# liuzuxin/OSRL

Measured on AMD Instinct MI355X. Metric: grad-steps/sec, higher is better.
Workload: dtype f32

## Files before the change

### osrl_amd/csrc/dwt.h

```cpp
#pragma once
#include "mlp_common.h"

namespace {

template <int T>
struct DwFragT {
  f32x4 a[T], b[T];
};

template <int T>
__device__ __forceinline__ void dwt_load(DwFragT<T>& f, const float* __restrict__ pz, const float* __restrict__ pa,
                                         size_t ldz, size_t lda_g, const unsigned (&oa)[T], const unsigned (&ia)[T],
                                         int nob, int nib) {
#pragma unroll
  for (int t = 0; t < 4; ++t) {
#pragma unroll
    for (int ob = 0; ob < T; ++ob) f.a[ob][t] = pz[t * ldz + oa[ob]];
#pragma unroll
    for (int ib = 0; ib < T; ++ib) f.b[ib][t] = pa[t * lda_g + ia[ib]];
  }
}
template <int T>
__device__ __forceinline__ void dwt_load_tail(DwFragT<T>& f, const float* __restrict__ dz, const float* __restrict__ av,
                                              size_t ldz, size_t lda_g, const unsigned (&oa)[T], const unsigned (&ia)[T],
                                              int nob, int nib, int r0, int r_end, int kq) {
#pragma unroll
  for (int t = 0; t < 4; ++t) {
    const int r = r0 + 4 * kq + t;
    const bool rok = r < r_end;
    const size_t rc = (size_t)(rok ? r : r_end - 1);
#pragma unroll
    for (int ob = 0; ob < T; ++ob) {
      const float v = dz[rc * ldz + oa[ob]];
      f.a[ob][t] = rok ? v : 0.f;
    }
#pragma unroll
    for (int ib = 0; ib < T; ++ib) f.b[ib][t] = av[rc * lda_g + ia[ib]];
  }
}

template <int T, int SHAPE>
__device__ __forceinline__ void dwt_mma(f32x4 (&acc)[T][T], float (&dbacc)[T], const DwFragT<T>& f, int nob, int nib,
                                        bool want_db) {
  constexpr bool FULL = SHAPE == 1;
#pragma unroll
  for (int t = 0; t < 4; ++t) {
#pragma unroll
    for (int ob = 0; ob < (SHAPE == 2 ? 1 : T); ++ob) {
      if (SHAPE != 0 || ob < nob) {
#pragma unroll
        for (int ib = 0; ib < T; ++ib)
          if (SHAPE != 0 || ib < nib) acc[ob][ib] = __builtin_amdgcn_mfma_f32_16x16x4f32(f.a[ob][t], f.b[ib][t], acc[ob][ib], 0, 0, 0);
      }
    }
  }
  (void)FULL;
  if (want_db) {
#pragma unroll
    for (int ob = 0; ob < T; ++ob) dbacc[ob] += (f.a[ob][0] + f.a[ob][1]) + (f.a[ob][2] + f.a[ob][3]);
  }
}

template <int T>
constexpr size_t dwt_lds() { return sizeof(float) * (4 * (16 * T) * (16 * T + 1) + 4 * 16 * T); }

template <int T, bool WARM = false, bool DEEP = false, class EPI>
__device__ __forceinline__ void dwt_tile(const osrl_dw_entry_t* __restrict__ entries, const int32_t* __restrict__ items,
                                         const int item, const int rows, float* __restrict__ red, EPI epi) {
  constexpr int TW = 16 * T, LD = TW + 1;
  const int tid = threadIdx.x, lane = tid & 63;
  const int wave = __builtin_amdgcn_readfirstlane(tid >> 6);
  const int ei = items[item * 4 + 0], ot = items[item * 4 + 1], it = items[item * 4 + 2], sp = items[item * 4 + 3];
  const int s = sp & 0xffff, nsp = sp >> 16;
  const OSRL_CAS osrl_dw_entry_t& E = ((const OSRL_CAS osrl_dw_entry_t*)entries)[ei];
  const int out = E.out, in = E.in;
  const size_t ldz = E.ldz > 0 ? (size_t)E.ldz : (size_t)out, lda_g = E.lda > 0 ? (size_t)E.lda : (size_t)in;
  const int o0 = ot * TW, i0 = it * TW;
  int rps = (rows + nsp - 1) / nsp;
  rps = (rps + 63) & ~63;
  const int rpw = rps >> 2;
  const int r_begin = s * rps + wave * rpw;
  int r_end = r_begin + rpw;
  r_end = r_end > rows ? rows : r_end;
  const int m = lane & 15, kq = lane >> 4;
  int nob = (out - o0 + 15) >> 4;
  nob = nob > T ? T : nob;
  int nib = (in - i0 + 15) >> 4;
  nib = nib > T ? T : nib;
  const bool want_db = it == 0;

  if (wave < 4) {
  f32x4 acc[T][T];
  zero_acc<T, T>(acc);
  float dbacc[T];
#pragma unroll
  for (int ob = 0; ob < T; ++ob) dbacc[ob] = 0.f;
  const float* __restrict__ dz = E.dz;
  const float* __restrict__ av = E.a;
  unsigned oa[T], ia[T];
#pragma unroll
  for (int b = 0; b < T; ++b) {
    const int o = o0 + b * 16 + m, i = i0 + b * 16 + m;
    oa[b] = (unsigned)(o < out ? o : 0);
    ia[b] = (unsigned)(i < in ? i : 0);
  }
  if (r_begin < r_end) {
    const int n_full = (r_end - r_begin) >> 4;
    const float* __restrict__ pz = dz + (size_t)(r_begin + 4 * kq) * ldz;
    const float* __restrict__ pa = av + (size_t)(r_begin + 4 * kq) * lda_g;
    float wt[WARM ? 4 * ((TW + 31) / 32) : 1];
    if constexpr (WARM) {
      constexpr int NL = (TW + 31) / 32;
#pragma unroll
      for (int pass = 0; pass < 2; ++pass) {
        int r = r_begin + pass * 64 + lane;
        r = r < r_end ? r : r_end - 1;
#pragma unroll
        for (int j = 0; j < NL; ++j) {
          const int oc = o0 + 32 * j < out ? o0 + 32 * j : out - 1, ic = i0 + 32 * j < in ? i0 + 32 * j : in - 1;
          wt[(pass * 2 + 0) * NL + j] = dz[(size_t)r * ldz + oc];
          wt[(pass * 2 + 1) * NL + j] = av[(size_t)r * lda_g + ic];
        }
      }
    }
    DwFragT<T> f0, f1;
    auto run = [&](auto full_c) {
      constexpr int FULL = decltype(full_c)::value;
      if constexpr (DEEP) {
        if (n_full == 4 && r_begin + 64 == r_end) {
          DwFragT<T> f2, f3;
          dwt_load<T>(f0, pz, pa, ldz, lda_g, oa, ia, nob, nib);
          dwt_load<T>(f1, pz + (size_t)16 * ldz, pa + (size_t)16 * lda_g, ldz, lda_g, oa, ia, nob, nib);
          dwt_load<T>(f2, pz + (size_t)32 * ldz, pa + (size_t)32 * lda_g, ldz, lda_g, oa, ia, nob, nib);
          dwt_load<T>(f3, pz + (size_t)48 * ldz, pa + (size_t)48 * lda_g, ldz, lda_g, oa, ia, nob, nib);
          dwt_mma<T, FULL>(acc, dbacc, f0, nob, nib, want_db);
          dwt_mma<T, FULL>(acc, dbacc, f1, nob, nib, want_db);
          dwt_mma<T, FULL>(acc, dbacc, f2, nob, nib, want_db);
          dwt_mma<T, FULL>(acc, dbacc, f3, nob, nib, want_db);
          return;
        }
      }
      if (n_full > 0) dwt_load<T>(f0, pz, pa, ldz, lda_g, oa, ia, nob, nib);
      int k = 0;
      for (; k + 1 < n_full; k += 2) {
        dwt_load<T>(f1, pz + (size_t)(k + 1) * 16 * ldz, pa + (size_t)(k + 1) * 16 * lda_g, ldz, lda_g, oa, ia, nob, nib);
        dwt_mma<T, FULL>(acc, dbacc, f0, nob, nib, want_db);
        const int kn = k + 2 < n_full ? k + 2 : n_full - 1;
        dwt_load<T>(f0, pz + (size_t)kn * 16 * ldz, pa + (size_t)kn * 16 * lda_g, ldz, lda_g, oa, ia, nob, nib);
        dwt_mma<T, FULL>(acc, dbacc, f1, nob, nib, want_db);
      }
      if (k < n_full) dwt_mma<T, FULL>(acc, dbacc, f0, nob, nib, want_db);
      if (r_begin + 16 * n_full < r_end) {
        dwt_load_tail<T>(f1, dz, av, ldz, lda_g, oa, ia, nob, nib, r_begin + 16 * n_full, r_end, kq);
        dwt_mma<T, FULL>(acc, dbacc, f1, nob, nib, want_db);
      }
    };
    if (nob == T && nib == T)
      run(std::integral_constant<int, 1>{});
    else if (nob == 1 && nib == T)
      run(std::integral_constant<int, 2>{});
    else
      run(std::integral_constant<int, 0>{});
    if constexpr (WARM) {
#pragma unroll
      for (int j = 0; j < 4 * ((TW + 31) / 32); ++j) asm volatile("" ::"v"(wt[j]));
    }
  }
  float* mine = red + wave * TW * LD;
#pragma unroll
  for (int ob = 0; ob < T; ++ob)
#pragma unroll
    for (int ib = 0; ib < T; ++ib)
#pragma unroll
      for (int r = 0; r < 4; ++r) mine[(ob * 16 + kq * 4 + r) * LD + ib * 16 + m] = acc[ob][ib][r];
  if (want_db) {
#pragma unroll
    for (int ob = 0; ob < T; ++ob) {
      float v = dbacc[ob];
      v += __shfl_xor(v, 16);
      v += __shfl_xor(v, 32);
      if (kq == 0) red[4 * TW * LD + wave * TW + ob * 16 + m] = v;
    }
  }
  }
  __syncthreads();
  epi(E, o0, i0, sp, want_db);
}

}
```

### osrl_amd/csrc/mlp_dw.hip

```cpp
#include "dwt.h"
#include "adam.h"
#include "trace.h"

namespace {

constexpr int kDwLd = 65;
constexpr size_t kDwLds = sizeof(float) * (4 * 64 * kDwLd + 4 * 64);

struct DwFrag {
  f32x4 a[4], b[4];
};

__device__ __forceinline__ void dw_load(DwFrag& f, const float* __restrict__ dz, const float* __restrict__ av,
                                        size_t ldz, size_t lda_g, int r0, int r_end, int o0, int i0, int out, int in,
                                        int nob, int nib, int m, int kq) {
#pragma unroll
  for (int t = 0; t < 4; ++t) {
    const int r = r0 + 4 * kq + t;
    const bool rok = r < r_end;
    const size_t rc = (size_t)(rok ? r : r_end - 1);
#pragma unroll
    for (int ob = 0; ob < 4; ++ob) {
      const int o = o0 + ob * 16 + m;
      const bool ok = rok && ob < nob && o < out;
      const float v = dz[rc * ldz + (o < out ? o : 0)];
      f.a[ob][t] = ok ? v : 0.f;
    }
#pragma unroll
    for (int ib = 0; ib < 4; ++ib) {
      const int i = i0 + ib * 16 + m;
      const bool ok = rok && ib < nib && i < in;
      const float v = av[rc * lda_g + (i < in ? i : 0)];
      f.b[ib][t] = ok ? v : 0.f;
    }
  }
}

__device__ __forceinline__ void dw_mma(f32x4 (&acc)[4][4], float (&dbacc)[4], const DwFrag& f, int nob, int nib,
                                       bool want_db) {
#pragma unroll
  for (int t = 0; t < 4; ++t) {
#pragma unroll
    for (int ob = 0; ob < 4; ++ob) {
      if (ob < nob) {
#pragma unroll
        for (int ib = 0; ib < 4; ++ib)
          if (ib < nib) acc[ob][ib] = __builtin_amdgcn_mfma_f32_16x16x4f32(f.a[ob][t], f.b[ib][t], acc[ob][ib], 0, 0, 0);
      }
    }
  }
  if (want_db) {
#pragma unroll
    for (int ob = 0; ob < 4; ++ob) dbacc[ob] += (f.a[ob][0] + f.a[ob][1]) + (f.a[ob][2] + f.a[ob][3]);
  }
}

__global__ __launch_bounds__(256) void mlp_dw_kernel(const osrl_dw_entry_t* __restrict__ entries,
                                                      const int32_t* __restrict__ items, int n_items, int rows,
                                                      int rows_per_split, float* __restrict__ slabs,
                                                      int64_t slab_stride) {
  extern __shared__ __attribute__((aligned(16))) float red[];
  const int tid = threadIdx.x, lane = tid & 63;
  const int wave = __builtin_amdgcn_readfirstlane(tid >> 6);
  const int item = blockIdx.x;
#if OSRL_CHAIN_PRIO > 0
  if (rows <= OSRL_CHAIN_PRIO) __builtin_amdgcn_s_setprio(3);
#endif
  const int ei = items[item * 4 + 0], ot = items[item * 4 + 1], it = items[item * 4 + 2];
  const osrl_dw_entry_t E = entries[ei];
  const int out = E.out, in = E.in;
  const size_t ldz = E.ldz > 0 ? (size_t)E.ldz : (size_t)out, lda_g = E.lda > 0 ? (size_t)E.lda : (size_t)in;
  const int o0 = ot * 64, i0 = it * 64;
  const int s = blockIdx.y;
  const int rpw = rows_per_split >> 2;
  const int r_begin = s * rows_per_split + wave * rpw;
  int r_end = r_begin + rpw;
  r_end = r_end > rows ? rows : r_end;
  const int m = lane & 15, kq = lane >> 4;
  int nob = (out - o0 + 15) >> 4;
  nob = nob > 4 ? 4 : nob;
  int nib = (in - i0 + 15) >> 4;
  nib = nib > 4 ? 4 : nib;
  const bool want_db = it == 0;

  f32x4 acc[4][4];
  zero_acc<4, 4>(acc);
  float dbacc[4] = {0.f, 0.f, 0.f, 0.f};
  const float* __restrict__ dz = E.dz;
  const float* __restrict__ av = E.a;
  if (r_begin < r_end) {
    DwFrag f0, f1;
    dw_load(f0, dz, av, ldz, lda_g, r_begin, r_end, o0, i0, out, in, nob, nib, m, kq);
    for (int r0 = r_begin; r0 < r_end; r0 += 32) {
      if (r0 + 16 < r_end) dw_load(f1, dz, av, ldz, lda_g, r0 + 16, r_end, o0, i0, out, in, nob, nib, m, kq);
      dw_mma(acc, dbacc, f0, nob, nib, want_db);
      if (r0 + 16 < r_end) {
        if (r0 + 32 < r_end) dw_load(f0, dz, av, ldz, lda_g, r0 + 32, r_end, o0, i0, out, in, nob, nib, m, kq);
        dw_mma(acc, dbacc, f1, nob, nib, want_db);
      }
    }
  }
  float* mine = red + wave * 64 * kDwLd;
#pragma unroll
  for (int ob = 0; ob < 4; ++ob)
#pragma unroll
    for (int ib = 0; ib < 4; ++ib)
#pragma unroll
      for (int r = 0; r < 4; ++r) mine[(ob * 16 + kq * 4 + r) * kDwLd + ib * 16 + m] = acc[ob][ib][r];
  if (want_db) {
#pragma unroll
    for (int ob = 0; ob < 4; ++ob) {
      float v = dbacc[ob];
      v += __shfl_xor(v, 16);
      v += __shfl_xor(v, 32);
      if (kq == 0) red[4 * 64 * kDwLd + wave * 64 + ob * 16 + m] = v;
    }
  }
  __syncthreads();
  float* __restrict__ slab = slabs + (size_t)s * slab_stride;
  const int il = tid & 63;
#pragma unroll 4
  for (int ol = tid >> 6; ol < 64; ol += 4) {
    const int off = ol * kDwLd + il;
    const float v = ((red[off] + red[64 * kDwLd + off]) + red[2 * 64 * kDwLd + off]) + red[3 * 64 * kDwLd + off];
    const int o = o0 + ol, i = i0 + il;
    if (o < out && i < in) slab[E.w_off + (size_t)o * in + i] = v;
  }
  if (want_db && tid < 64) {
    const float* db = red + 4 * 64 * kDwLd;
    const float v = ((db[tid] + db[64 + tid]) + db[128 + tid]) + db[192 + tid];
    if (o0 + tid < out) slab[E.b_off + o0 + tid] = v;
  }
}


template <int T>
__global__ __launch_bounds__(256, 1) void mlp_dwt_kernel(const osrl_dw_entry_t* __restrict__ entries,
                                                         const int32_t* __restrict__ items, int rows,
                                                         float* __restrict__ slabs, int64_t slab_stride) {
  extern __shared__ __attribute__((aligned(16))) float red[];
  constexpr int TW = 16 * T, LD = TW + 1;
  const int tid = threadIdx.x;
  OSRL_TRACE_BEGIN(100 + T, entries);
#if OSRL_CHAIN_PRIO > 0
  if (rows <= OSRL_CHAIN_PRIO) __builtin_amdgcn_s_setprio(3);
#endif
  dwt_tile<T>(entries, items, blockIdx.x, rows, red,
              [&](const OSRL_CAS osrl_dw_entry_t& E, const int o0, const int i0, const int sp, const bool want_db) {
    const int out = E.out, in = E.in;
    float* __restrict__ slab = slabs + (size_t)(sp & 0xffff) * slab_stride;
    for (int idx = tid; idx < TW * TW; idx += 256) {
      const int ol = idx / TW, il = idx - ol * TW;
      const int off = ol * LD + il;
      const float v = ((red[off] + red[TW * LD + off]) + red[2 * TW * LD + off]) + red[3 * TW * LD + off];
      const int o = o0 + ol, i = i0 + il;
      if (o < out && i < in) slab[E.w_off + (size_t)o * in + i] = v;
    }
    if (want_db && tid < TW) {
      const float* db = red + 4 * TW * LD;
      const float v = ((db[tid] + db[TW + tid]) + db[2 * TW + tid]) + db[3 * TW + tid];
      if (o0 + tid < out) slab[E.b_off + o0 + tid] = v;
    }
  });
}




struct DwAdamArgs {
  const osrl_dw_entry_t* entries;
  const int32_t* items;
  const int32_t* tile_ids;
  uint32_t* counters;
  float* slabs;
  int64_t slab_stride;
  float *p, *m, *v, *tgt;
  const int32_t *map_f, *map_b;
  float *pf, *pb, *tf;
  const osrl_step_state_t* st;
  float lr, b1, b2, eps, tau;
  int32_t rows, pad_;
};

__device__ __forceinline__ void slab_put(float* p, float v) {
  __hip_atomic_store(p, v, __ATOMIC_RELAXED, __HIP_MEMORY_SCOPE_AGENT);
}
__device__ __forceinline__ float slab_get(const float* p) {
  return __hip_atomic_load(p, __ATOMIC_RELAXED, __HIP_MEMORY_SCOPE_AGENT);
}

template <int T, class AR>
__device__ __forceinline__ void mlp_dwt_adam_body(AR a) {
  extern __shared__ __attribute__((aligned(16))) float red[];
  __shared__ int s_last;
  constexpr int TW = 16 * T, LD = TW + 1;
  constexpr int PER = (TW * TW + 255) / 256;
  const int tid = threadIdx.x;
  const int rows = a.rows;
#if OSRL_CHAIN_PRIO > 0
  if (rows <= OSRL_CHAIN_PRIO) __builtin_amdgcn_s_setprio(3);
#endif
  const int item = blockIdx.x;
  dwt_tile<T>(a.entries, a.items, item, rows, red,
              [&](const OSRL_CAS osrl_dw_entry_t& E, const int o0, const int i0, const int sp, const bool want_db) {
    const int out = E.out, in = E.in;
    const int s = sp & 0xffff, nsp = sp >> 16;
    float* __restrict__ slabs = a.slabs;
    const int64_t stride = a.slab_stride;
    const int64_t w_off = E.w_off, b_off = E.b_off;
    float* __restrict__ P = a.p;
    float* __restrict__ M = a.m;
    float* __restrict__ V = a.v;
    float* TG = a.tgt;
    const int32_t* MF = a.map_f;
    const int32_t* MB = a.map_b;
    const float* TGr = TG ? TG : P;
    const int32_t* MFr = MF ? MF : reinterpret_cast<const int32_t*>(P);
    const int32_t* MBr = MB ? MB : reinterpret_cast<const int32_t*>(P);
    unsigned w[PER];
    bool ok[PER];
    int offl[PER];
    float pv[PER], mv[PER], vv[PER], tv0[PER];
    int mf[PER], mb[PER];
#pragma unroll
    for (int j = 0; j < PER; ++j) {
      const int idx = tid + j * 256;
      const int ol = idx / TW, il = idx - ol * TW;
      const int o = o0 + ol, i = i0 + il;
      ok[j] = idx < TW * TW && o < out && i < in;
      w[j] = (unsigned)(ok[j] ? w_off + (int64_t)o * in + i : w_off);
      offl[j] = ok[j] ? ol * LD + il : 0;
      pv[j] = P[w[j]];
      mv[j] = M[w[j]];
      vv[j] = V[w[j]];
      tv0[j] = TGr[w[j]];
      mf[j] = MFr[w[j]];
      mb[j] = MBr[w[j]];
    }
    const bool has_b = want_db && tid < TW && o0 + tid < out;
    const unsigned wb = (unsigned)(b_off + (has_b ? o0 + tid : 0));
    float pb_ = P[wb], mb_ = M[wb], vb_ = V[wb], tb_ = TGr[wb];
    if (nsp > 1) {
      float* __restrict__ slab = slabs + (size_t)s * stride;
#pragma unroll
      for (int j = 0; j < PER; ++j) {
        const int off = offl[j];
        const float v = ((red[off] + red[TW * LD + off]) + red[2 * TW * LD + off]) + red[3 * TW * LD + off];
        if (ok[j]) slab_put(slab + w[j], v);
      }
      if (has_b) {
        const float* db = red + 4 * TW * LD;
        slab_put(slab + wb, ((db[tid] + db[TW + tid]) + db[2 * TW + tid]) + db[3 * TW + tid]);
      }
      asm volatile("s_waitcnt vmcnt(0)" ::: "memory");
      __syncthreads();
      if (tid == 0) {
        unsigned* c = a.counters + a.tile_ids[item];
        const unsigned seen = __hip_atomic_fetch_add(c, 1u, __ATOMIC_RELAXED, __HIP_MEMORY_SCOPE_AGENT);
        const int last = seen == (unsigned)nsp - 1;
        if (last) __hip_atomic_store(c, 0u, __ATOMIC_RELAXED, __HIP_MEMORY_SCOPE_AGENT);
        s_last = last;
      }
      __syncthreads();
      if (!s_last) return;
    }
    const osrl_step_state_t* __restrict__ st = a.st;
    const float lr_t = a.lr * st->lr_scale;
    const osrl_adam::Coef c{a.b1, a.b2, a.eps, lr_t / st->bc1, st->bc2_sqrt};
    const float tau = a.tau;
    auto apply = [&](const unsigned wi, const float g, float p_, float m_, float v_, const float t0, const int mfi,
                     const int mbi) {
      osrl_adam::update1(p_, m_, v_, g, c);
      P[wi] = p_;
      M[wi] = m_;
      V[wi] = v_;
      float tv = p_;
      if (TG) {
        tv = osrl_adam::polyak1(tau, p_, t0);
        TG[wi] = tv;
      }
      if (MF && mfi >= 0) {
        a.pf[mfi] = p_;
        if (TG && a.tf) a.tf[mfi] = tv;
      }
      if (MF && MB && mbi >= 0) a.pb[mbi] = p_;
    };
    float g[PER], gb = 0.f;
    if (nsp > 1) {
      auto gather = [&](auto ks_c) {
        constexpr int KS = decltype(ks_c)::value;
        float sl[PER][KS], sb[KS];
#pragma unroll
        for (int j = 0; j < PER; ++j)
#pragma unroll
          for (int q = 0; q < KS; ++q) sl[j][q] = slab_get(slabs + (size_t)(q < nsp ? q : 0) * stride + w[j]);
#pragma unroll
        for (int q = 0; q < KS; ++q) sb[q] = slab_get(slabs + (size_t)(q < nsp ? q : 0) * stride + wb);
#pragma unroll
        for (int j = 0; j < PER; ++j) {
          g[j] = sl[j][0];
#pragma unroll
          for (int q = 1; q < KS; ++q)
            if (q < nsp) g[j] += sl[j][q];
          for (int q = KS; q < nsp; ++q) g[j] += slab_get(slabs + (size_t)q * stride + w[j]);
        }
        gb = sb[0];
#pragma unroll
        for (int q = 1; q < KS; ++q)
          if (q < nsp) gb += sb[q];
        for (int q = KS; q < nsp; ++q) gb += slab_get(slabs + (size_t)q * stride + wb);
      };
      if (nsp <= 4 || PER > 16)
        gather(std::integral_constant<int, 4>{});
      else
        gather(std::integral_constant<int, 8>{});
    } else {
#pragma unroll
      for (int j = 0; j < PER; ++j) {
        const int off = offl[j];
        g[j] = ((red[off] + red[TW * LD + off]) + red[2 * TW * LD + off]) + red[3 * TW * LD + off];
      }
      const float* db = red + 4 * TW * LD;
      const int tb = has_b ? tid : 0;
      gb = ((db[tb] + db[TW + tb]) + db[2 * TW + tb]) + db[3 * TW + tb];
    }
#pragma unroll
    for (int j = 0; j < PER; ++j)
      if (ok[j]) apply(w[j], g[j], pv[j], mv[j], vv[j], tv0[j], mf[j], mb[j]);
    if (has_b) apply(wb, gb, pb_, mb_, vb_, tb_, -1, -1);
  });
}
template <int T>
__global__ __launch_bounds__(256, 1) void mlp_dwt_adam_kernel(const DwAdamArgs a) {
  mlp_dwt_adam_body<T, const DwAdamArgs&>(a);
}
template <int T>
__global__ __launch_bounds__(256, 1) void mlp_dwt_adam_kernel_p(const void* p) {
  mlp_dwt_adam_body<T, const OSRL_CAS DwAdamArgs&>(*(const OSRL_CAS DwAdamArgs*)p);
}


constexpr int kDwbO = 8, kDwbI = 4;

struct DwBigFrag {
  f32x4 a[kDwbO], b[kDwbI];
};

template <bool GUARD>
__device__ __forceinline__ void dwp_load(DwBigFrag& f, const float* __restrict__ dz, const float* __restrict__ av,
                                         size_t ldz, size_t lda_g, int r0, int r_end, int m, int kq) {
#pragma unroll
  for (int t = 0; t < 4; ++t) {
    const int r = r0 + 4 * kq + t;
    const bool rok = !GUARD || r < r_end;
    const size_t rc = (size_t)(rok ? r : r_end - 1);
    const float* __restrict__ pz = dz + rc * ldz + 4 * m;
    const float* __restrict__ pa = av + rc * lda_g + 4 * m;
#pragma unroll
    for (int q = 0; q < kDwbO / 4; ++q) {
      const f32x4 v = *reinterpret_cast<const f32x4*>(pz + 64 * q);
#pragma unroll
      for (int j = 0; j < 4; ++j) f.a[4 * q + j][t] = rok ? v[j] : 0.f;
    }
#pragma unroll
    for (int q = 0; q < kDwbI / 4; ++q) {
      const f32x4 v = *reinterpret_cast<const f32x4*>(pa + 64 * q);
#pragma unroll
      for (int j = 0; j < 4; ++j) f.b[4 * q + j][t] = rok ? v[j] : 0.f;
    }
  }
}

__global__ __launch_bounds__(256, 1) void mlp_dw_big_kernel(const osrl_dw_entry_t* __restrict__ entries,
                                                    const int32_t* __restrict__ items, int n_items, int rows,
                                                    int rows_per_split, float* __restrict__ slabs, int64_t slab_stride) {
  const int lane = threadIdx.x & 63;
  const int wave = __builtin_amdgcn_readfirstlane(threadIdx.x >> 6);
  const int item = blockIdx.x * 4 + wave;
  if (item >= n_items) return;
  const int ei = items[item * 4 + 0], ot = items[item * 4 + 1], it = items[item * 4 + 2];
  const osrl_dw_entry_t E = entries[ei];
  const int out = E.out, in = E.in;
  const size_t ldz = E.ldz > 0 ? (size_t)E.ldz : (size_t)out, lda_g = E.lda > 0 ? (size_t)E.lda : (size_t)in;
  const int o0 = ot * 16 * kDwbO, i0 = it * 16 * kDwbI;
  const int s = blockIdx.y;
  const int r_begin = s * rows_per_split;
  int r_end = r_begin + rows_per_split;
  r_end = r_end > rows ? rows : r_end;
  const int m = lane & 15, kq = lane >> 4;
  const bool want_db = it == 0;
  const float* __restrict__ dz = E.dz + o0;
  const float* __restrict__ av = E.a + i0;
  f32x4 acc[kDwbO][kDwbI];
#pragma unroll
  for (int ob = 0; ob < kDwbO; ++ob)
#pragma unroll
    for (int ib = 0; ib < kDwbI; ++ib) acc[ob][ib] = f32x4{0.f, 0.f, 0.f, 0.f};
  float dbacc[kDwbO];
#pragma unroll
  for (int ob = 0; ob < kDwbO; ++ob) dbacc[ob] = 0.f;
  auto mma = [&](const DwBigFrag& f) __attribute__((always_inline)) {
#pragma unroll
    for (int t = 0; t < 4; ++t)
#pragma unroll
      for (int ob = 0; ob < kDwbO; ++ob)
#pragma unroll
        for (int ib = 0; ib < kDwbI; ++ib)
          acc[ob][ib] = __builtin_amdgcn_mfma_f32_16x16x4f32(f.a[ob][t], f.b[ib][t], acc[ob][ib], 0, 0, 0);
    if (want_db) {
#pragma unroll
      for (int ob = 0; ob < kDwbO; ++ob) dbacc[ob] += (f.a[ob][0] + f.a[ob][1]) + (f.a[ob][2] + f.a[ob][3]);
    }
  };
  if (r_begin < r_end) {
    DwBigFrag f[2];
    const int n_steps = (r_end - r_begin + 15) >> 4;
    const int n_full = (r_end - r_begin) >> 4;
    const float* pz = dz + (size_t)(r_begin + 4 * kq) * ldz + 4 * m;
    const float* pa = av + (size_t)(r_begin + 4 * kq) * lda_g + 4 * m;
    const size_t zstep = 16 * ldz, astep = 16 * lda_g;
    auto load_fast = [&](DwBigFrag& g) __attribute__((always_inline)) {
#pragma unroll
      for (int t = 0; t < 4; ++t) {
#pragma unroll
        for (int q = 0; q < kDwbO / 4; ++q) {
          const f32x4 v = *reinterpret_cast<const f32x4*>(pz + t * ldz + 64 * q);
#pragma unroll
          for (int j = 0; j < 4; ++j) g.a[4 * q + j][t] = v[j];
        }
#pragma unroll
        for (int q = 0; q < kDwbI / 4; ++q) {
          const f32x4 v = *reinterpret_cast<const f32x4*>(pa + t * lda_g + 64 * q);
#pragma unroll
          for (int j = 0; j < 4; ++j) g.b[4 * q + j][t] = v[j];
        }
      }
      pz += zstep;
      pa += astep;
    };
    int st = 0;
    if (n_full >= 1) load_fast(f[0]);
    else dwp_load<true>(f[0], dz, av, ldz, lda_g, r_begin, r_end, m, kq);
    while (st + 3 <= n_full) {
      load_fast(f[1]);
      mma(f[0]);
      __builtin_amdgcn_sched_group_barrier(0x020, 12, 0);
      __builtin_amdgcn_sched_group_barrier(0x008, 4 * kDwbO * kDwbI, 0);
      load_fast(f[0]);
      mma(f[1]);
      __builtin_amdgcn_sched_group_barrier(0x020, 12, 0);
      __builtin_amdgcn_sched_group_barrier(0x008, 4 * kDwbO * kDwbI, 0);
      st += 2;
    }
    while (st < n_steps) {
      if ((st & 1) == 0) {
        dwp_load<true>(f[1], dz, av, ldz, lda_g, r_begin + 16 * (st + 1), r_end, m, kq);
        mma(f[0]);
      } else {
        dwp_load<true>(f[0], dz, av, ldz, lda_g, r_begin + 16 * (st + 1), r_end, m, kq);
        mma(f[1]);
      }
      ++st;
    }
  }
  float* __restrict__ slab = slabs + (size_t)s * slab_stride;
#pragma unroll
  for (int ob = 0; ob < kDwbO; ++ob)
#pragma unroll
    for (int qb = 0; qb < kDwbI / 4; ++qb)
#pragma unroll
      for (int r = 0; r < 4; ++r) {
        const int orow = o0 + 64 * (ob >> 2) + 4 * (4 * kq + r) + (ob & 3);
        const f32x4 v = {acc[ob][4 * qb + 0][r], acc[ob][4 * qb + 1][r], acc[ob][4 * qb + 2][r], acc[ob][4 * qb + 3][r]};
        *reinterpret_cast<f32x4*>(&slab[E.w_off + (size_t)orow * in + i0 + 64 * qb + 4 * m]) = v;
      }
  if (want_db) {
#pragma unroll
    for (int ob = 0; ob < kDwbO; ++ob) {
      float v = dbacc[ob];
      v += __shfl_xor(v, 16);
      v += __shfl_xor(v, 32);
      if (kq == 0) slab[E.b_off + o0 + 64 * (ob >> 2) + 4 * m + (ob & 3)] = v;
    }
  }
}


constexpr int kCoS = 4;
__device__ __forceinline__ void dwc_glds16(const void* g, float* lds_wave_base) {
  __builtin_amdgcn_global_load_lds((const __attribute__((address_space(1))) void*)g,
                                   (__attribute__((address_space(3))) void*)lds_wave_base, 16, 0, 0);
}
__global__ __launch_bounds__(512, 2) void mlp_dw_coop_kernel(const osrl_dw_entry_t* __restrict__ entries,
                                                  const int32_t* __restrict__ items, int n_items, int rows,
                                                  int rows_per_split, float* __restrict__ slabs, int64_t slab_stride) {
  extern __shared__ __attribute__((aligned(16))) float lds_co[];
  constexpr int kSlot = 2 * 16 * 256;
  const int tid = threadIdx.x, lane = tid & 63;
  const int wave = __builtin_amdgcn_readfirstlane(tid >> 6);
  const int wo = wave >> 2, wi = wave & 3;
  const int item = blockIdx.x;
  const int ei = items[item * 4 + 0], ot = items[item * 4 + 1], it = items[item * 4 + 2];
  const osrl_dw_entry_t E = entries[ei];
  const int out = E.out, in = E.in;
  const size_t ldz = E.ldz > 0 ? (size_t)E.ldz : (size_t)out, lda_g = E.lda > 0 ? (size_t)E.lda : (size_t)in;
  const int o0 = ot * 256, i0 = it * 256;
  const int s = blockIdx.y;
  const int r_begin = s * rows_per_split;
  int r_end = r_begin + rows_per_split;
  r_end = r_end > rows ? rows : r_end;
  const int m = lane & 15, kq = lane >> 4;
  const bool want_db = it == 0 && wi == 0;
  const int G = (r_end - r_begin) >> 4;
  f32x4 acc[kDwbO][kDwbI];
#pragma unroll
  for (int ob = 0; ob < kDwbO; ++ob)
#pragma unroll
    for (int ib = 0; ib < kDwbI; ++ib) acc[ob][ib] = f32x4{0.f, 0.f, 0.f, 0.f};
  float dbacc[kDwbO];
#pragma unroll
  for (int ob = 0; ob < kDwbO; ++ob) dbacc[ob] = 0.f;
  if (G > 0) {
    const char* src[4];
    size_t step_b[4];
    int dst_off[4];
#pragma unroll
    for (int p = 0; p < 4; ++p) {
      const int idx = 4 * wave + p, mat = idx >> 4, row = idx & 15;
      const float* base = mat ? E.a + i0 : E.dz + o0;
      const size_t ld = mat ? lda_g : ldz;
      src[p] = reinterpret_cast<const char*>(base + (size_t)(r_begin + row) * ld + 4 * lane);
      step_b[p] = 16 * ld * sizeof(float);
      dst_off[p] = mat * 16 * 256 + row * 256;
    }
    int it_slot = 0, it_g = 0;
    auto dma = [&]() __attribute__((always_inline)) {
      if (it_g < G) {
#pragma unroll
        for (int p = 0; p < 4; ++p) {
          dwc_glds16(src[p], lds_co + it_slot * kSlot + dst_off[p]);
          src[p] += step_b[p];
        }
      }
      ++it_g;
      it_slot = it_slot + 1 == kCoS ? 0 : it_slot + 1;
    };
    const int z_off = (4 * kq) * 256 + wo * 128 + 4 * m;
    const int a_off = 16 * 256 + (4 * kq) * 256 + wi * 64 + 4 * m;
    DwBigFrag f;
    auto rd = [&](int slot, DwBigFrag& g) __attribute__((always_inline)) {
      const float* sl = lds_co + slot * kSlot;
#pragma unroll
      for (int t = 0; t < 4; ++t) {
#pragma unroll
        for (int q = 0; q < kDwbO / 4; ++q) {
          const f32x4 v = *reinterpret_cast<const f32x4*>(sl + z_off + t * 256 + 64 * q);
#pragma unroll
          for (int j = 0; j < 4; ++j) g.a[4 * q + j][t] = v[j];
        }
        const f32x4 v = *reinterpret_cast<const f32x4*>(sl + a_off + t * 256);
#pragma unroll
        for (int j = 0; j < 4; ++j) g.b[j][t] = v[j];
      }
    };
    auto mma_t = [&](const DwBigFrag& g, int t) __attribute__((always_inline)) {
#pragma unroll
      for (int ob = 0; ob < kDwbO; ++ob)
#pragma unroll
        for (int ib = 0; ib < kDwbI; ++ib)
          acc[ob][ib] = __builtin_amdgcn_mfma_f32_16x16x4f32(g.a[ob][t], g.b[ib][t], acc[ob][ib], 0, 0, 0);
    };
    constexpr int L = kCoS - 1, DMA_OPS = 4;
#pragma unroll
    for (int i = 0; i < L; ++i) dma();
    int c_slot = 0;
    for (int g = 0; g < G; ++g) {
      if (g + L <= G) asm volatile("s_waitcnt vmcnt(%0)\n\ts_barrier" ::"n"((L - 1) * DMA_OPS) : "memory");
      else asm volatile("s_waitcnt vmcnt(0)\n\ts_barrier" ::: "memory");
      rd(c_slot, f);
      c_slot = c_slot + 1 == kCoS ? 0 : c_slot + 1;
#pragma unroll
      for (int t = 0; t < 4; ++t) {
        if ((t == 0 && wo == 0) || (t == 2 && wo == 1)) dma();
        mma_t(f, t);
      }
      if (want_db) {
#pragma unroll
        for (int ob = 0; ob < kDwbO; ++ob) dbacc[ob] += (f.a[ob][0] + f.a[ob][1]) + (f.a[ob][2] + f.a[ob][3]);
      }
      __builtin_amdgcn_sched_barrier(0);
    }
    asm volatile("s_waitcnt vmcnt(0)" ::: "memory");
  }
  float* __restrict__ slab = slabs + (size_t)s * slab_stride;
  const int ow = o0 + wo * 128, iw = i0 + wi * 64;
#pragma unroll
  for (int ob = 0; ob < kDwbO; ++ob)
#pragma unroll
    for (int r = 0; r < 4; ++r) {
      const int orow = ow + 64 * (ob >> 2) + 4 * (4 * kq + r) + (ob & 3);
      const f32x4 v = {acc[ob][0][r], acc[ob][1][r], acc[ob][2][r], acc[ob][3][r]};
      *reinterpret_cast<f32x4*>(&slab[E.w_off + (size_t)orow * in + iw + 4 * m]) = v;
    }
  if (want_db) {
#pragma unroll
    for (int ob = 0; ob < kDwbO; ++ob) {
      float v = dbacc[ob];
      v += __shfl_xor(v, 16);
      v += __shfl_xor(v, 32);
      if (kq == 0) slab[E.b_off + ow + 64 * (ob >> 2) + 4 * m + (ob & 3)] = v;
    }
  }
}

}

extern "C" int osrl_mlp_backward_dw_big(const osrl_dw_entry_t* d_entries, const int32_t* d_items, int32_t n_items,
                                        int32_t rows, int32_t n_splits, float* slabs, int64_t slab_stride,
                                        void* stream) {
  if (!d_entries || !d_items || n_items < 1 || rows < 1 || n_splits < 1 || !slabs) return -1;
  int rps = (rows + n_splits - 1) / n_splits;
  rps = (rps + 15) & ~15;
  constexpr int kLds = 96 * 1024;
  hipError_t e = hipFuncSetAttribute(reinterpret_cast<const void*>(mlp_dw_big_kernel),
                                     hipFuncAttributeMaxDynamicSharedMemorySize, kLds);
  if (e != hipSuccess) return (int)e;
  (void)hipGetLastError();
  hipLaunchKernelGGL(mlp_dw_big_kernel, dim3((n_items + 3) / 4, n_splits, 1), dim3(256), kLds, (hipStream_t)stream,
                     d_entries, d_items, n_items, rows, rps, slabs, slab_stride);
  return (int)hipGetLastError();
}

extern "C" int osrl_mlp_backward_dw_coop(const osrl_dw_entry_t* d_entries, const int32_t* d_items, int32_t n_items,
                                         int32_t rows, int32_t n_splits, float* slabs, int64_t slab_stride,
                                         void* stream) {
  if (!d_entries || !d_items || n_items < 1 || rows < 16 || (rows & 15) || n_splits < 1 || !slabs) return -1;
  int rps = (rows + n_splits - 1) / n_splits;
  rps = (rps + 15) & ~15;
  constexpr int kLds = sizeof(float) * kCoS * 2 * 16 * 256;
  hipError_t e = hipFuncSetAttribute(reinterpret_cast<const void*>(mlp_dw_coop_kernel),
                                     hipFuncAttributeMaxDynamicSharedMemorySize, kLds);
  if (e != hipSuccess) return (int)e;
  (void)hipGetLastError();
  hipLaunchKernelGGL(mlp_dw_coop_kernel, dim3(n_items, n_splits, 1), dim3(512), kLds, (hipStream_t)stream, d_entries,
                     d_items, n_items, rows, rps, slabs, slab_stride);
  return (int)hipGetLastError();
}

template <int T>
static int launch_dwt(const osrl_dw_entry_t* d_entries, const int32_t* d_items, int32_t n_work, int32_t rows, float* slabs,
                      int64_t slab_stride, hipStream_t stream) {
  hipError_t e = hipFuncSetAttribute(reinterpret_cast<const void*>(mlp_dwt_kernel<T>),
                                     hipFuncAttributeMaxDynamicSharedMemorySize, (int)dwt_lds<T>());
  if (e != hipSuccess) return (int)e;
  (void)hipGetLastError();
  hipLaunchKernelGGL(mlp_dwt_kernel<T>, dim3(n_work), dim3(256), dwt_lds<T>(), stream, d_entries, d_items, rows, slabs,
                     slab_stride);
  return (int)hipGetLastError();
}

extern "C" int osrl_mlp_backward_dw_tiles(const osrl_dw_entry_t* d_entries, const int32_t* d_work, int32_t n_work,
                                          int32_t rows, int32_t tile_blocks, float* slabs, int64_t slab_stride,
                                          void* stream) {
  if (!d_entries || !d_work || n_work < 1 || rows < 1 || !slabs) return -1;
  (void)hipGetLastError();
  if (tile_blocks == 5) return launch_dwt<5>(d_entries, d_work, n_work, rows, slabs, slab_stride, (hipStream_t)stream);
  if (tile_blocks == 4) return launch_dwt<4>(d_entries, d_work, n_work, rows, slabs, slab_stride, (hipStream_t)stream);
  if (tile_blocks == 3) return launch_dwt<3>(d_entries, d_work, n_work, rows, slabs, slab_stride, (hipStream_t)stream);
  if (tile_blocks == 2) return launch_dwt<2>(d_entries, d_work, n_work, rows, slabs, slab_stride, (hipStream_t)stream);
  return -1;
}

template <int T>
static int launch_dwt_adam(const DwAdamArgs& a, int32_t n_work, hipStream_t stream) {
  return osrl_argmem::launch(mlp_dwt_adam_kernel<T>, mlp_dwt_adam_kernel_p<T>, dim3(n_work), dim3(256), dwt_lds<T>(), stream, a);
}

extern "C" int osrl_mlp_backward_dw_tiles_adam(const osrl_dw_entry_t* d_entries, const int32_t* d_work,
                                               const int32_t* d_tile_ids, uint32_t* d_counters, int32_t n_work,
                                               int32_t rows, int32_t tile_blocks, float* slabs, int64_t slab_stride,
                                               const osrl_dw_adam_t* o, void* stream) {
  if (!d_entries || !d_work || !d_tile_ids || !d_counters || n_work < 1 || rows < 1 || !slabs || !o) return -1;
  if (!o->p || !o->m || !o->v || !o->st || (o->map_f && !o->pf) || (o->map_b && (!o->pb || !o->map_f))) return -1;
  DwAdamArgs a{};
  a.entries = d_entries;
  a.items = d_work;
  a.tile_ids = d_tile_ids;
  a.counters = d_counters;
  a.slabs = slabs;
  a.slab_stride = slab_stride;
  a.p = o->p; a.m = o->m; a.v = o->v; a.tgt = o->tgt;
  a.map_f = o->map_f; a.map_b = o->map_b;
  a.pf = o->pf; a.pb = o->pb; a.tf = o->tgt ? o->tf : nullptr;
  a.st = o->st;
  a.lr = o->lr; a.b1 = o->beta1; a.b2 = o->beta2; a.eps = o->eps; a.tau = o->tau;
  a.rows = rows;
  (void)hipGetLastError();
  hipStream_t st = (hipStream_t)stream;
  if (tile_blocks == 5) return launch_dwt_adam<5>(a, n_work, st);
  if (tile_blocks == 4) return launch_dwt_adam<4>(a, n_work, st);
  if (tile_blocks == 3) return launch_dwt_adam<3>(a, n_work, st);
  if (tile_blocks == 2) return launch_dwt_adam<2>(a, n_work, st);
  return -1;
}

extern "C" int osrl_mlp_backward_dw(const osrl_dw_entry_t* d_entries, const int32_t* d_items, int32_t n_items,
                                    int32_t rows, int32_t n_splits, float* slabs, int64_t slab_stride,
                                    void* stream) {
  if (!d_entries || !d_items || n_items < 1 || rows < 1 || n_splits < 1 || !slabs) return -1;
  int rps = (rows + n_splits - 1) / n_splits;
  rps = (rps + 63) & ~63;
  dim3 grid(n_items, n_splits, 1);
  (void)hipGetLastError();
  hipError_t e = hipFuncSetAttribute(reinterpret_cast<const void*>(mlp_dw_kernel),
                                     hipFuncAttributeMaxDynamicSharedMemorySize, (int)kDwLds);
  if (e != hipSuccess) return (int)e;
  (void)hipGetLastError();
  hipLaunchKernelGGL(mlp_dw_kernel, grid, dim3(256), kDwLds, (hipStream_t)stream, d_entries, d_items, n_items, rows,
                     rps, slabs, slab_stride);
  return (int)hipGetLastError();
}
```

Measured before the change: 2683.

## Vectorize dW tile global loads with permuted column mapping and tune launch bounds

Adds a wide-load path to the weight-gradient tile kernel. Each lane now owns V adjacent columns instead of columns strided by 16, so dz and activation fragments can be fetched with float2/float4 loads. The LDS reduction store and the bias index are permuted to match the new column mapping. The path is used only for full, aligned tiles and can be disabled with OSRL_DW_WIDE=0. The launch bounds for T=2 also change to a minimum of 3 workgroups, which may constrain register allocation.

```diff
diff --git a/osrl_amd/csrc/dwt.h b/osrl_amd/csrc/dwt.h
--- a/osrl_amd/csrc/dwt.h
+++ b/osrl_amd/csrc/dwt.h
@@ -36,6 +36,53 @@
     }
 #pragma unroll
     for (int ib = 0; ib < T; ++ib) f.b[ib][t] = av[rc * lda_g + ia[ib]];
+  }
+}
+
+template <int T>
+struct DwWide {
+  static constexpr int V = T >= 4 ? 4 : (T >= 2 ? 2 : 1);
+  static constexpr int NV = (T / V) * V;
+};
+typedef float dwt_f32x2 __attribute__((ext_vector_type(2)));
+template <int T>
+__device__ __forceinline__ int dwt_col(const int b, const int m, const bool wide) {
+  constexpr int V = DwWide<T>::V, NV = DwWide<T>::NV;
+  return (wide && b < NV) ? (b / V) * 16 * V + V * m + (b % V) : b * 16 + m;
+}
+template <int T, bool WA, bool WB>
+__device__ __forceinline__ void dwt_load_w(DwFragT<T>& f, const float* __restrict__ pz, const float* __restrict__ pa,
+                                           size_t ldz, size_t lda_g, const unsigned (&oa)[T], const unsigned (&ia)[T]) {
+  constexpr int V = DwWide<T>::V, NV = DwWide<T>::NV;
+  using VT = std::conditional_t<V == 4, f32x4, dwt_f32x2>;
+#pragma unroll
+  for (int t = 0; t < 4; ++t) {
+    if constexpr (WA && V > 1) {
+#pragma unroll
+      for (int q = 0; q < NV / V; ++q) {
+        const VT v = *reinterpret_cast<const VT*>(pz + t * ldz + oa[q * V]);
+#pragma unroll
+        for (int j = 0; j < V; ++j) f.a[q * V + j][t] = v[j];
+      }
+#pragma unroll
+      for (int ob = NV; ob < T; ++ob) f.a[ob][t] = pz[t * ldz + oa[ob]];
+    } else {
+#pragma unroll
+      for (int ob = 0; ob < T; ++ob) f.a[ob][t] = pz[t * ldz + oa[ob]];
+    }
+    if constexpr (WB && V > 1) {
+#pragma unroll
+      for (int q = 0; q < NV / V; ++q) {
+        const VT v = *reinterpret_cast<const VT*>(pa + t * lda_g + ia[q * V]);
+#pragma unroll
+        for (int j = 0; j < V; ++j) f.b[q * V + j][t] = v[j];
+      }
+#pragma unroll
+      for (int ib = NV; ib < T; ++ib) f.b[ib][t] = pa[t * lda_g + ia[ib]];
+    } else {
+#pragma unroll
+      for (int ib = 0; ib < T; ++ib) f.b[ib][t] = pa[t * lda_g + ia[ib]];
+    }
   }
 }
 
@@ -64,9 +111,10 @@
 template <int T>
 constexpr size_t dwt_lds() { return sizeof(float) * (4 * (16 * T) * (16 * T + 1) + 4 * 16 * T); }
 
-template <int T, bool WARM = false, bool DEEP = false, class EPI>
+template <int T, bool WARM = false, bool DEEP = false, bool WIDE_OK = false, class EPI>
 __device__ __forceinline__ void dwt_tile(const osrl_dw_entry_t* __restrict__ entries, const int32_t* __restrict__ items,
-                                         const int item, const int rows, float* __restrict__ red, EPI epi) {
+                                         const int item, const int rows, float* __restrict__ red, EPI epi,
+                                         const int wide = 0) {
   constexpr int TW = 16 * T, LD = TW + 1;
   const int tid = threadIdx.x, lane = tid & 63;
   const int wave = __builtin_amdgcn_readfirstlane(tid >> 6);
@@ -97,10 +145,18 @@
   for (int ob = 0; ob < T; ++ob) dbacc[ob] = 0.f;
   const float* __restrict__ dz = E.dz;
   const float* __restrict__ av = E.a;
+  constexpr int WV = DwWide<T>::V, WNV = DwWide<T>::NV;
+  bool wa = false, wb = false;
+  if constexpr (WIDE_OK && WV > 1) {
+    const bool full = wide != 0 && nob == T && nib == T;
+    wa = full && o0 + 16 * WNV <= out && (ldz & (WV - 1)) == 0 && ((uintptr_t)dz & (4 * WV - 1)) == 0;
+    wb = full && i0 + 16 * WNV <= in && (lda_g & (WV - 1)) == 0 && ((uintptr_t)av & (4 * WV - 1)) == 0;
+    wa = wb = wa && wb;
+  }
   unsigned oa[T], ia[T];
 #pragma unroll
   for (int b = 0; b < T; ++b) {
-    const int o = o0 + b * 16 + m, i = i0 + b * 16 + m;
+    const int o = o0 + dwt_col<T>(b, m, wa), i = i0 + dwt_col<T>(b, m, wb);
     oa[b] = (unsigned)(o < out ? o : 0);
     ia[b] = (unsigned)(i < in ? i : 0);
   }
@@ -124,8 +180,13 @@
       }
     }
     DwFragT<T> f0, f1;
-    auto run = [&](auto full_c) {
+    auto run = [&](auto full_c, auto wide_c) {
       constexpr int FULL = decltype(full_c)::value;
+      constexpr bool WA = (decltype(wide_c)::value & 1) != 0, WB = (decltype(wide_c)::value & 2) != 0;
+      auto load = [&](DwFragT<T>& f, const float* __restrict__ z, const float* __restrict__ x) __attribute__((always_inline)) {
+        if constexpr (WA || WB) dwt_load_w<T, WA, WB>(f, z, x, ldz, lda_g, oa, ia);
+        else dwt_load<T>(f, z, x, ldz, lda_g, oa, ia, nob, nib);
+      };
       if constexpr (DEEP) {
         if (n_full == 4 && r_begin + 64 == r_end) {
           DwFragT<T> f2, f3;
@@ -140,13 +201,13 @@
           return;
         }
       }
-      if (n_full > 0) dwt_load<T>(f0, pz, pa, ldz, lda_g, oa, ia, nob, nib);
+      if (n_full > 0) load(f0, pz, pa);
       int k = 0;
       for (; k + 1 < n_full; k += 2) {
-        dwt_load<T>(f1, pz + (size_t)(k + 1) * 16 * ldz, pa + (size_t)(k + 1) * 16 * lda_g, ldz, lda_g, oa, ia, nob, nib);
+        load(f1, pz + (size_t)(k + 1) * 16 * ldz, pa + (size_t)(k + 1) * 16 * lda_g);
         dwt_mma<T, FULL>(acc, dbacc, f0, nob, nib, want_db);
         const int kn = k + 2 < n_full ? k + 2 : n_full - 1;
-        dwt_load<T>(f0, pz + (size_t)kn * 16 * ldz, pa + (size_t)kn * 16 * lda_g, ldz, lda_g, oa, ia, nob, nib);
+        load(f0, pz + (size_t)kn * 16 * ldz, pa + (size_t)kn * 16 * lda_g);
         dwt_mma<T, FULL>(acc, dbacc, f1, nob, nib, want_db);
       }
       if (k < n_full) dwt_mma<T, FULL>(acc, dbacc, f0, nob, nib, want_db);
@@ -155,31 +216,49 @@
         dwt_mma<T, FULL>(acc, dbacc, f1, nob, nib, want_db);
       }
     };
-    if (nob == T && nib == T)
-      run(std::integral_constant<int, 1>{});
-    else if (nob == 1 && nib == T)
-      run(std::integral_constant<int, 2>{});
+    using NoWide = std::integral_constant<int, 0>;
+    if (nob == T && nib == T) {
+      if (wa && wb)
+        run(std::integral_constant<int, 1>{}, std::integral_constant<int, 3>{});
+      else
+        run(std::integral_constant<int, 1>{}, NoWide{});
+    } else if (nob == 1 && nib == T)
+      run(std::integral_constant<int, 2>{}, NoWide{});
     else
-      run(std::integral_constant<int, 0>{});
+      run(std::integral_constant<int, 0>{}, NoWide{});
     if constexpr (WARM) {
 #pragma unroll
       for (int j = 0; j < 4 * ((TW + 31) / 32); ++j) asm volatile("" ::"v"(wt[j]));
     }
   }
   float* mine = red + wave * TW * LD;
-#pragma unroll
-  for (int ob = 0; ob < T; ++ob)
-#pragma unroll
-    for (int ib = 0; ib < T; ++ib)
-#pragma unroll
-      for (int r = 0; r < 4; ++r) mine[(ob * 16 + kq * 4 + r) * LD + ib * 16 + m] = acc[ob][ib][r];
+  auto put = [&](auto w_c) __attribute__((always_inline)) {
+    constexpr bool W = decltype(w_c)::value;
+    constexpr int V = W ? DwWide<T>::V : 1, NV = W ? DwWide<T>::NV : 0;
+    float* const b_nn = mine + (4 * kq) * LD + m;
+    float* const b_nw = mine + (4 * kq) * LD + V * m;
+    float* const b_wn = mine + (V * 4 * kq) * LD + m;
+    float* const b_ww = mine + (V * 4 * kq) * LD + V * m;
+#pragma unroll
+    for (int ob = 0; ob < T; ++ob)
+#pragma unroll
+      for (int ib = 0; ib < T; ++ib) {
+        float* const base = ob < NV ? (ib < NV ? b_ww : b_wn) : (ib < NV ? b_nw : b_nn);
+#pragma unroll
+        for (int r = 0; r < 4; ++r) base[dwt_col<T>(ob, r, W) * LD + dwt_col<T>(ib, 0, W)] = acc[ob][ib][r];
+      }
+  };
+  if (wa)
+    put(std::true_type{});
+  else
+    put(std::false_type{});
   if (want_db) {
 #pragma unroll
     for (int ob = 0; ob < T; ++ob) {
       float v = dbacc[ob];
       v += __shfl_xor(v, 16);
       v += __shfl_xor(v, 32);
-      if (kq == 0) red[4 * TW * LD + wave * TW + ob * 16 + m] = v;
+      if (kq == 0) red[4 * TW * LD + wave * TW + dwt_col<T>(ob, m, wa)] = v;
     }
   }
   }
diff --git a/osrl_amd/csrc/mlp_dw.hip b/osrl_amd/csrc/mlp_dw.hip
--- a/osrl_amd/csrc/mlp_dw.hip
+++ b/osrl_amd/csrc/mlp_dw.hip
@@ -135,9 +135,12 @@
 
 
 template <int T>
-__global__ __launch_bounds__(256, 1) void mlp_dwt_kernel(const osrl_dw_entry_t* __restrict__ entries,
+constexpr int dwt_min_wg() { return T == 2 ? 3 : 1; }
+
+template <int T>
+__global__ __launch_bounds__(256, dwt_min_wg<T>()) void mlp_dwt_kernel(const osrl_dw_entry_t* __restrict__ entries,
                                                          const int32_t* __restrict__ items, int rows,
-                                                         float* __restrict__ slabs, int64_t slab_stride) {
+                                                         float* __restrict__ slabs, int64_t slab_stride, int wide) {
   extern __shared__ __attribute__((aligned(16))) float red[];
   constexpr int TW = 16 * T, LD = TW + 1;
   const int tid = threadIdx.x;
@@ -145,7 +148,7 @@
 #if OSRL_CHAIN_PRIO > 0
   if (rows <= OSRL_CHAIN_PRIO) __builtin_amdgcn_s_setprio(3);
 #endif
-  dwt_tile<T>(entries, items, blockIdx.x, rows, red,
+  dwt_tile<T, false, false, true>(entries, items, blockIdx.x, rows, red,
               [&](const OSRL_CAS osrl_dw_entry_t& E, const int o0, const int i0, const int sp, const bool want_db) {
     const int out = E.out, in = E.in;
     float* __restrict__ slab = slabs + (size_t)(sp & 0xffff) * slab_stride;
@@ -161,7 +164,7 @@
       const float v = ((db[tid] + db[TW + tid]) + db[2 * TW + tid]) + db[3 * TW + tid];
       if (o0 + tid < out) slab[E.b_off + o0 + tid] = v;
     }
-  });
+  }, wide);
 }
 
 
@@ -179,7 +182,7 @@
   float *pf, *pb, *tf;
   const osrl_step_state_t* st;
   float lr, b1, b2, eps, tau;
-  int32_t rows, pad_;
+  int32_t rows, wide;
 };
 
 __device__ __forceinline__ void slab_put(float* p, float v) {
@@ -201,7 +204,7 @@
   if (rows <= OSRL_CHAIN_PRIO) __builtin_amdgcn_s_setprio(3);
 #endif
   const int item = blockIdx.x;
-  dwt_tile<T>(a.entries, a.items, item, rows, red,
+  dwt_tile<T, false, false, true>(a.entries, a.items, item, rows, red,
               [&](const OSRL_CAS osrl_dw_entry_t& E, const int o0, const int i0, const int sp, const bool want_db) {
     const int out = E.out, in = E.in;
     const int s = sp & 0xffff, nsp = sp >> 16;
@@ -328,14 +331,14 @@
     for (int j = 0; j < PER; ++j)
       if (ok[j]) apply(w[j], g[j], pv[j], mv[j], vv[j], tv0[j], mf[j], mb[j]);
     if (has_b) apply(wb, gb, pb_, mb_, vb_, tb_, -1, -1);
-  });
+  }, a.wide);
 }
 template <int T>
-__global__ __launch_bounds__(256, 1) void mlp_dwt_adam_kernel(const DwAdamArgs a) {
+__global__ __launch_bounds__(256, dwt_min_wg<T>()) void mlp_dwt_adam_kernel(const DwAdamArgs a) {
   mlp_dwt_adam_body<T, const DwAdamArgs&>(a);
 }
 template <int T>
-__global__ __launch_bounds__(256, 1) void mlp_dwt_adam_kernel_p(const void* p) {
+__global__ __launch_bounds__(256, dwt_min_wg<T>()) void mlp_dwt_adam_kernel_p(const void* p) {
   mlp_dwt_adam_body<T, const OSRL_CAS DwAdamArgs&>(*(const OSRL_CAS DwAdamArgs*)p);
 }
 
@@ -647,6 +650,11 @@
   return (int)hipGetLastError();
 }
 
+inline int dw_wide_env() {
+  const char* v = getenv("OSRL_DW_WIDE");
+  return (v && v[0] == '0') ? 0 : 1;
+}
+
 template <int T>
 static int launch_dwt(const osrl_dw_entry_t* d_entries, const int32_t* d_items, int32_t n_work, int32_t rows, float* slabs,
                       int64_t slab_stride, hipStream_t stream) {
@@ -655,7 +663,7 @@
   if (e != hipSuccess) return (int)e;
   (void)hipGetLastError();
   hipLaunchKernelGGL(mlp_dwt_kernel<T>, dim3(n_work), dim3(256), dwt_lds<T>(), stream, d_entries, d_items, rows, slabs,
-                     slab_stride);
+                     slab_stride, dw_wide_env());
   return (int)hipGetLastError();
 }
 
@@ -695,6 +703,7 @@
   a.st = o->st;
   a.lr = o->lr; a.b1 = o->beta1; a.b2 = o->beta2; a.eps = o->eps; a.tau = o->tau;
   a.rows = rows;
+  a.wide = dw_wide_env();
   (void)hipGetLastError();
   hipStream_t st = (hipStream_t)stream;
   if (tile_blocks == 5) return launch_dwt_adam<5>(a, n_work, st);
```

After: 2693 (median of 6 runs). No clear change (+0.4%).
